# ethz-asl/object_keypoints

Measured on AMD Instinct MI355X. Metric: frames/sec keypoint inference (511x511 -> heatmaps+3D), higher is better.
Workload: dtype bf16; 1 GPU; BASELINE configs[2]: batch=64/GPU synthetic 511x511 frames, bf16 activations+weights, fp32 accumulate, CornerNet-Squeeze K=3 (valve) random-init procedural weights; fp32 NCHW frames -> stem -> hourglass+heads; peak-NMS -> depth lifting -> object grouping on injected bump scenes (SURVEY 8(d), 1-2 objects/frame); frames_per_gpu=64, global_batch=64, parallelism=frame-dp1, resident_frame_batches=4

## Files before the change

object_keypoints_amd/csrc/okp_igemm_patch.hip:

```cpp
#include <cstdio>
#include <cstdlib>
#include <cstring>
#include <type_traits>
#include <vector>

#include "okp_igemm_kernel.h"


namespace {

constexpr uint32_t kPatchKeys = 0x7ac788u;
template <int MT> __device__ __forceinline__ uint32_t patch_key(int col) {
  return MT == 16 ? (kPatchKeys >> (3 * (col >> 1))) & 7u : (uint32_t)(col >> 1) & 7u;
}

constexpr int kWStage = 256 * 128;
constexpr int kPitch = 18;
constexpr int kPatchBuf = 41 * 1024;
constexpr int kLdsPatch = 2 * kWStage;
constexpr int kLdsSteps = kLdsPatch + 2 * kPatchBuf;
constexpr int kLdsBias = kLdsSteps + 256 * (int)sizeof(OkpPatchStep);
#ifdef OKP_PATCH_STAMPS
constexpr int kStampBytes = 1024;
__device__ __forceinline__ uint64_t stamp() { uint64_t t; asm volatile("s_memtime %0" : "=s"(t)); return t; }
#else
constexpr int kStampBytes = 0;
#endif
constexpr int kGeoEntries = 328;
constexpr int kLdsGeo = kLdsBias + 1024;
constexpr int kLdsStamps = kLdsGeo + OKP_PATCH_MAX_GEOM * kGeoEntries * 4;
constexpr int kLdsTotal = kLdsStamps + kStampBytes;
static_assert(sizeof(OkpPatchStep) == 16, "step table entries are read as one 16-byte vector");
static_assert(256 * 512 <= kLdsSteps, "epilogue staging (256 px x 256 ch bf16) must not reach the step table");
static_assert(kLdsTotal <= 160 * 1024, "one workgroup's LDS is at most the CU's 160 KiB");

template <typename T, int MT = 16, bool RG = false>
__global__ __launch_bounds__(512) void okp_igemm_patch_kernel(const OkpPatchParams p) {
  static_assert(!RG || std::is_same<T, _Float16>::value, "the 16-bit storage guard is an fp16 instantiation");
  using x4_t = typename H16<T>::x4;
  using x8_t = typename H16<T>::x8;
  static_assert(MT == 16 || MT == 32, "MFMA tile");
  constexpr int TCO = 64 / MT, TPX = 128 / MT;
  constexpr int AREGS = MT * MT / 64;
  using acc_t = typename Mma<T, MT>::acc_t;
  __shared__ __attribute__((aligned(16))) char smem[kLdsTotal];
  char* const steps_lds = smem + kLdsSteps;
  char* const bias_lds = smem + kLdsBias;

  const int tid = threadIdx.x;
  const int lane = tid & 63;
  const int wave = __builtin_amdgcn_readfirstlane(tid >> 6);
  const int wco = wave >> 1, wpx = wave & 1;
  const int fr = lane & 15, fh = lane >> 4;

  const __amdgpu_buffer_rsrc_t rs_w = __builtin_amdgcn_make_buffer_rsrc(const_cast<void*>(p.weights), 0, (int)p.w_bytes, 0x00020000);
  const __amdgpu_buffer_rsrc_t rs_b = __builtin_amdgcn_make_buffer_rsrc(const_cast<float*>(p.bias), 0, p.n_co_tiles * 256 * 4, 0x00020000);
  const __amdgpu_buffer_rsrc_t rs_s0 = __builtin_amdgcn_make_buffer_rsrc(const_cast<void*>(p.src_data[0]), 0, (int)p.src_bytes[0], 0x00020000);
  const __amdgpu_buffer_rsrc_t rs_s1 = __builtin_amdgcn_make_buffer_rsrc(const_cast<void*>(p.src_data[1]), 0, (int)p.src_bytes[1], 0x00020000);

  if (tid < p.n_steps) reinterpret_cast<u32x4*>(steps_lds)[tid] = reinterpret_cast<const u32x4*>(p.steps)[tid];
  __syncthreads();

  const int r0 = tid >> 3;
  const int wc = (tid & 7) ^ ((r0 >> 1) & 7);

  for (int slot = blockIdx.x; slot < p.n_tiles; slot += gridDim.x) {
    const int xq = p.n_tiles >> 3, xr = p.n_tiles & 7, xcd = slot & 7;
    const int tile = (xcd < xr ? xcd * (xq + 1) : xr * (xq + 1) + (xcd - xr) * xq) + (slot >> 3);
    const int cls = p.n_classes == 4 ? (tile & 3) : 0;
    const int tile_c = p.n_classes == 4 ? (tile >> 2) : tile;
    const int t0 = cls * p.steps_per_class, t1 = t0 + p.steps_per_class;
    const int co_tile = tile_c % p.n_co_tiles;
    const int px_tile = tile_c / p.n_co_tiles;
    const int n = fastdiv(px_tile, p.div_tiles_frame);
    const int trem = px_tile - n * p.tiles_y * p.tiles_x;
    const int tyi = fastdiv(trem, p.div_tiles_x);
    const int y0 = tyi * 16, x0 = (trem - tyi * p.tiles_x) * 16;
    const int co0 = co_tile * 256;

    if (wave == 0)
      __builtin_amdgcn_raw_ptr_buffer_load_lds(rs_b, (lds_ptr_t)bias_lds, 16, (int)((uint32_t)(co0 + lane * 4) * 4u), 0, 0, 0);

    uint32_t wbase[4];
#pragma unroll
    for (int i = 0; i < 4; ++i) {
      const int co = co0 + r0 + i * 64;
      wbase[i] = (co < p.cout_pad) ? (uint32_t)co * 128u + (uint32_t)wc * 16u : kInvalidOff;
    }

    auto issue_w = [&](int t, int stage) {
      const uint32_t wslice = (uint32_t)t * (uint32_t)p.cout_pad * 128u;
      char* const wt = smem + stage * kWStage + wave * 1024;
#pragma unroll
      for (int i = 0; i < 4; ++i)
        __builtin_amdgcn_raw_ptr_buffer_load_lds(rs_w, (lds_ptr_t)(wt + i * 8192), 16, (int)(wbase[i] + wslice), 0, 0, 0);
    };
    auto patch_pixel = [&](const OkpPatchGeom& G, int idx) -> uint32_t {
      const int i = idx / kPitch, j = idx - i * kPitch;
      const int ys = G.conv_stride * y0 + G.oy + i * G.step, xs = G.conv_stride * x0 + G.ox + j * G.step;
      const bool ok = idx < G.npx && j < G.PW && ys >= 0 && ys < G.H && xs >= 0 && xs < G.W;
      return ok ? ((uint32_t)((n * G.H + ys) * G.W + xs) * (uint32_t)(G.pix_stride * 2)) | patch_key<MT>(j) : kInvalidOff;
    };
    auto issue_patch_tab = [&](int geom, uint32_t c0b, int k0, int k1, int buf) {
      const int npx = 18 * (int)((p.geom_ph >> (5 * geom)) & 31u);
      const __amdgpu_buffer_rsrc_t rs_x = ((p.geom_src >> geom) & 1) ? rs_s1 : rs_s0;
      const uint32_t* const tab = reinterpret_cast<const uint32_t*>(smem + kLdsGeo) + geom * kGeoEntries + (lane >> 3);
      for (int k = k0; k < k1; ++k) {
        const int blk = k * 8 + wave;
        if (blk * 8 >= npx) continue;
        const uint32_t e = tab[blk * 8];
        const uint32_t off = (e & kInvalidOff) ? kInvalidOff : (e & ~7u) + c0b + ((((uint32_t)lane & 7u) ^ (e & 7u)) << 4);
        __builtin_amdgcn_raw_ptr_buffer_load_lds(rs_x, (lds_ptr_t)(smem + kLdsPatch + buf * kPatchBuf + blk * 1024), 16, (int)off, 0, 0, 0);
      }
    };
    auto issue_patch = [&](int geom, uint32_t c0b, int k0, int k1, int buf) {
      const OkpPatchGeom& G = p.g[geom];
      const int PW = G.PW, npx = G.npx;
      const int H = G.H, W = G.W, ps2 = G.pix_stride * 2, step = G.step;
      const int yb = G.conv_stride * y0 + G.oy, xb = G.conv_stride * x0 + G.ox;
      const __amdgpu_buffer_rsrc_t rs_x = __builtin_amdgcn_make_buffer_rsrc(const_cast<void*>(G.data), 0, (int)G.bytes, 0x00020000);
      for (int k = k0; k < k1; ++k) {
        const int blk = k * 8 + wave;
        if (blk * 8 >= npx) continue;
        const int idx = blk * 8 + (lane >> 3);
        const int i = idx / kPitch, j = idx - i * kPitch;
        const int ch = (lane & 7) ^ (int)patch_key<MT>(j);
        const int ys = yb + i * step, xs = xb + j * step;
        const bool ok = idx < npx && j < PW && ys >= 0 && ys < H && xs >= 0 && xs < W;
        const uint32_t off = ok ? (uint32_t)((n * H + ys) * W + xs) * (uint32_t)ps2 + c0b + (uint32_t)ch * 16u : kInvalidOff;
        char* const dst = smem + kLdsPatch + buf * kPatchBuf + blk * 1024;
        __builtin_amdgcn_raw_ptr_buffer_load_lds(rs_x, (lds_ptr_t)dst, 16, (int)off, 0, 0, 0);
      }
    };

    acc_t acc[TCO][TPX];
#pragma unroll
    for (int i = 0; i < TCO; ++i)
#pragma unroll
      for (int j = 0; j < TPX; ++j)
#pragma unroll
        for (int e = 0; e < AREGS; ++e) acc[i][j][e] = 0.f;

    for (int g = 0; g < p.n_geom; ++g)
      if (tid < kGeoEntries) reinterpret_cast<uint32_t*>(smem + kLdsGeo)[g * kGeoEntries + tid] = patch_pixel(p.g[g], tid);
    {
      const u32x4 s0 = *reinterpret_cast<const u32x4*>(steps_lds + t0 * 16);
      const uint32_t w3 = (uint32_t)__builtin_amdgcn_readfirstlane((int)s0[3]);
      const int g0 = w3 & 0xff;
      issue_patch(g0, ((w3 >> 16) & 0xffu) * 128u, 0, (p.g[g0].npx + 63) >> 6, __builtin_amdgcn_readfirstlane((int)s0[2]) & 0xff);
    }
    issue_w(t0, t0 & 1);

    for (int t = t0; t < t1; ++t) {
      const u32x4 sv = *reinterpret_cast<const u32x4*>(steps_lds + t * 16);
      const uint32_t tap_bytes = (uint32_t)__builtin_amdgcn_readfirstlane((int)sv[0]);
      const uint32_t nx_c0b = (uint32_t)__builtin_amdgcn_readfirstlane((int)sv[1]);
      const uint32_t pk = (uint32_t)__builtin_amdgcn_readfirstlane((int)sv[2]);
      const int pbuf = pk & 0xff, nx_k0 = (pk >> 8) & 0xff, nx_k1 = (pk >> 16) & 0xff, nx_geom = pk >> 24;
      const uint32_t w3 = (uint32_t)__builtin_amdgcn_readfirstlane((int)sv[3]);
      const int dxo = (w3 >> 8) & 0xff;
      const bool more = t + 1 < t1;
#ifdef OKP_PATCH_ABL_NOPATCH
      const bool next_patch = false; (void)nx_k0; (void)nx_k1; (void)nx_geom; (void)nx_c0b;
#else
      const bool next_patch = nx_k1 > nx_k0 && (int)(w3 >> 24) + 1 < t1;
#endif

#ifdef OKP_PATCH_STAMPS
      uint64_t T0 = stamp();
      asm volatile("s_waitcnt vmcnt(0) lgkmcnt(0)" ::: "memory");
      uint64_t T1 = stamp();
      asm volatile("s_waitcnt lgkmcnt(0)" ::: "memory");
      __builtin_amdgcn_s_barrier();
      uint64_t T2 = stamp();
#else
      asm volatile("s_waitcnt vmcnt(0) lgkmcnt(0)" ::: "memory");
      __builtin_amdgcn_s_barrier();
#endif

      const char* const wt = smem + (t & 1) * kWStage;
      const char* const pbase = smem + kLdsPatch + pbuf * kPatchBuf;
      if constexpr (MT == 32) {
        const int r32 = lane & 31, h32 = lane >> 5;
        const char* const bb = pbase + tap_bytes + (uint32_t)(((wpx * 8 + (r32 >> 4)) * kPitch + (r32 & 15)) * 128);
        const uint32_t bsw = patch_key<32>((r32 & 15) + dxo);
        auto lda = [&](int sub, int i) { return *reinterpret_cast<const u32x4*>(wt + swz<128>((wco * TCO + i) * 32 + r32, 2 * sub + h32)); };
        auto ldb = [&](int sub, int j) { return *reinterpret_cast<const u32x4*>(bb + j * (2 * kPitch * 128) + ((((uint32_t)(2 * sub + h32)) ^ bsw) << 4)); };
        u32x4 fa[2][TCO], fb[2][TPX];
#pragma unroll
        for (int i = 0; i < TCO; ++i) fa[0][i] = lda(0, i);
#pragma unroll
        for (int j = 0; j < TPX; ++j) fb[0][j] = ldb(0, j);
        if (more) issue_w(t + 1, (t + 1) & 1);
#pragma unroll
        for (int sub = 0; sub < 4; ++sub) {
          __builtin_amdgcn_sched_barrier(0);
          if (sub + 1 < 4) {
#pragma unroll
            for (int i = 0; i < TCO; ++i) fa[(sub + 1) & 1][i] = lda(sub + 1, i);
#pragma unroll
            for (int j = 0; j < TPX; ++j) fb[(sub + 1) & 1][j] = ldb(sub + 1, j);
          }
          if (sub == 1 && next_patch) issue_patch_tab(nx_geom, nx_c0b, nx_k0, nx_k1, pbuf ^ 1);
          __builtin_amdgcn_sched_barrier(0);
#pragma unroll
          for (int i = 0; i < TCO; ++i)
#pragma unroll
            for (int j = 0; j < TPX; ++j) acc[i][j] = H16<T>::mfma32(fa[sub & 1][i], fb[sub & 1][j], acc[i][j]);
        }
      } else {
      const char* const bb = pbase + tap_bytes + (uint32_t)((wpx * TPX * kPitch + fr) * 128);
      const uint32_t bsw = patch_key<16>(fr + dxo);
      auto lda = [&](int kk, int i) {
        return *reinterpret_cast<const u32x4*>(wt + swz<128>((wco * TCO + i) * 16 + fr, 4 * kk + fh));
      };
      auto ldb = [&](int kk, int j) {
        return *reinterpret_cast<const u32x4*>(bb + j * (kPitch * 128) + ((((uint32_t)(4 * kk + fh)) ^ bsw) << 4));
      };
      auto mma8 = [&](const u32x4 (&a)[TCO], const u32x4 (&bq)[2], auto s) {
        constexpr int S = decltype(s)::value;
#pragma unroll
        for (int i = 0; i < TCO; ++i)
#pragma unroll
          for (int h = 0; h < 2; ++h)
            acc[i][2 * S + h] = H16<T>::mfma16(a[i], bq[h], acc[i][2 * S + h]);
      };
      using S0 = std::integral_constant<int, 0>; using S1 = std::integral_constant<int, 1>;
      using S2 = std::integral_constant<int, 2>; using S3 = std::integral_constant<int, 3>;
      u32x4 a0[TCO], a1[TCO], bq0[2], bq1[2];
#pragma unroll
      for (int i = 0; i < TCO; ++i) a0[i] = lda(0, i);
      bq0[0] = ldb(0, 0); bq0[1] = ldb(0, 1);
      bq1[0] = ldb(0, 2); bq1[1] = ldb(0, 3);
      if (more) issue_w(t + 1, (t + 1) & 1);
      __builtin_amdgcn_sched_barrier(0);
      mma8(a0, bq0, S0{});
      __builtin_amdgcn_sched_barrier(0);
#ifdef OKP_PATCH_STAMPS
      {
        uint64_t T3 = stamp();
        asm volatile("s_waitcnt lgkmcnt(0)" : "+s"(T0), "+s"(T1), "+s"(T2), "+s"(T3) :: "memory");
        if (slot == (int)blockIdx.x && lane == 0 && t - t0 < kStampBytes / 128)
          *reinterpret_cast<u32x4*>(smem + kLdsStamps + ((t - t0) * 8 + wave) * 16) = u32x4{(uint32_t)T0, (uint32_t)T1, (uint32_t)T2, (uint32_t)T3};
      }
      __builtin_amdgcn_sched_barrier(0);
#endif
      bq0[0] = ldb(0, 4); bq0[1] = ldb(0, 5); a1[0] = lda(1, 0); a1[1] = lda(1, 1);
      __builtin_amdgcn_sched_barrier(0);
      mma8(a0, bq1, S1{});
      __builtin_amdgcn_sched_barrier(0);
      bq1[0] = ldb(0, 6); bq1[1] = ldb(0, 7); a1[2] = lda(1, 2); a1[3] = lda(1, 3);
      __builtin_amdgcn_sched_barrier(0);
      mma8(a0, bq0, S2{});
      __builtin_amdgcn_sched_barrier(0);
      bq0[0] = ldb(1, 0); bq0[1] = ldb(1, 1);
      if (next_patch) issue_patch_tab(nx_geom, nx_c0b, nx_k0, nx_k1, pbuf ^ 1);
      __builtin_amdgcn_sched_barrier(0);
      mma8(a0, bq1, S3{});
      __builtin_amdgcn_sched_barrier(0);
      bq1[0] = ldb(1, 2); bq1[1] = ldb(1, 3);
      __builtin_amdgcn_sched_barrier(0);
      mma8(a1, bq0, S0{});
      __builtin_amdgcn_sched_barrier(0);
      bq0[0] = ldb(1, 4); bq0[1] = ldb(1, 5);
      __builtin_amdgcn_sched_barrier(0);
      mma8(a1, bq1, S1{});
      __builtin_amdgcn_sched_barrier(0);
      bq1[0] = ldb(1, 6); bq1[1] = ldb(1, 7);
      __builtin_amdgcn_sched_barrier(0);
      mma8(a1, bq0, S2{});
      mma8(a1, bq1, S3{});
          }
    }
#ifdef OKP_PATCH_STAMPS
    {
      uint64_t TE = stamp();
      asm volatile("s_waitcnt lgkmcnt(0)" : "+s"(TE) :: "memory");
      if (slot == (int)blockIdx.x && lane == 0 && t1 - t0 < kStampBytes / 128)
        *reinterpret_cast<u32x4*>(smem + kLdsStamps + ((t1 - t0) * 8 + wave) * 16) = u32x4{(uint32_t)TE, 0u, 0u, 0u};
    }
    __syncthreads();
    if (slot == (int)blockIdx.x && blockIdx.x < 16 && p.dbg)
      for (int i = tid; i < kStampBytes / 4; i += 512) p.dbg[blockIdx.x * (kStampBytes / 4) + i] = reinterpret_cast<const uint32_t*>(smem + kLdsStamps)[i];
#endif
    __syncthreads();

#pragma unroll
    for (int i = 0; i < TCO; ++i) {
#pragma unroll
      for (int g = 0; g < AREGS / 4; ++g) {
        const int co_l = (wco * TCO + i) * MT + (MT == 32 ? 8 * g + 4 * (lane >> 5) : 4 * fh);
        const f32x4 bv = *reinterpret_cast<const f32x4*>(bias_lds + co_l * 4);
#pragma unroll
        for (int j = 0; j < TPX; ++j) {
          const int prow = (wpx * TPX + j) * MT + (lane & (MT - 1));
          char* dst = smem + prow * 512 + ((((co_l * 2) >> 4) ^ (prow & 7)) << 4) + ((co_l * 2) & 15);
          x4_t o;
#pragma unroll
          for (int e = 0; e < 4; ++e) o[e] = (T)(acc[i][j][4 * g + e] + bv[e]);
          *reinterpret_cast<x4_t*>(dst) = o;
        }
      }
    }
    __syncthreads();
    constexpr int U = 256 * 32 / 512;
    constexpr int UH = 8;
    const bool relu = p.act == OKP_ACT_RELU;
    uint32_t range_h = 0u;
#pragma unroll 1
    for (int ub = 0; ub < U; ub += UH) {
      u32x4 rres[UH];
      uint32_t ooff[UH];
#pragma unroll
      for (int u = 0; u < UH; ++u) {
        const int it = tid + (ub + u) * 512;
        const int q = it & 31, prow = it >> 5;
        const int co = co0 + q * 8;
        const uint32_t opix = (uint32_t)((n * p.OH + (y0 + (prow >> 4)) * p.out_step + p.out_oy + (cls >> 1)) * p.OW + (x0 + (prow & 15)) * p.out_step + p.out_ox + (cls & 1));
        ooff[u] = co < p.cout ? opix : kInvalidOff;
      }
      if (p.res) {
#pragma unroll
        for (int u = 0; u < UH; ++u) {
          const int q = (tid + (ub + u) * 512) & 31;
          const int co = co0 + q * 8;
          const uint32_t opix = ooff[u] == kInvalidOff ? 0u : ooff[u];
          rres[u] = *reinterpret_cast<const u32x4*>(static_cast<const char*>(p.res) + ((size_t)opix * p.res_pix_stride + (co < p.cout ? co : 0)) * 2);
        }
      }
#pragma unroll
      for (int u = 0; u < UH; ++u) {
        const int it = tid + (ub + u) * 512;
        const int q = it & 31, prow = it >> 5;
        u32x4 w = *reinterpret_cast<const u32x4*>(smem + prow * 512 + ((q ^ (prow & 7)) << 4));
        if (ooff[u] == kInvalidOff) continue;
        char* op = static_cast<char*>(p.out) + ((size_t)ooff[u] * p.out_pix_stride + co0 + q * 8) * 2;
        if (!p.res) {
          if (relu) {
            typedef short s16x8 __attribute__((ext_vector_type(8)));
            const s16x8 z = {0, 0, 0, 0, 0, 0, 0, 0};
            w = __builtin_bit_cast(u32x4, __builtin_elementwise_max(__builtin_bit_cast(s16x8, w), z));
          }
          if constexpr (RG) range_h = okp_range_max_h8(range_h, w);
          *reinterpret_cast<u32x4*>(op) = w;
        } else {
          const x8_t s8 = __builtin_bit_cast(x8_t, w), r8 = __builtin_bit_cast(x8_t, rres[u]);
          x8_t o;
#pragma unroll
          for (int e = 0; e < 8; ++e) {
            float v = (float)s8[e] + (float)r8[e];
            if (relu) v = fmaxf(v, 0.f);
            o[e] = (T)v;
          }
          if constexpr (RG) range_h = okp_range_max_h8(range_h, __builtin_bit_cast(u32x4, o));
          *reinterpret_cast<x8_t*>(op) = o;
        }
      }
    }
    if constexpr (RG) okp_raise_range_flag(p.range_flag, okp_range_exceeded_h2(range_h));
    __syncthreads();
  }
}

}

bool okp_patch_supported(const okp_conv* plan, const OkpIgemmParams& p) {
  const bool x3 = plan->dtype == OKP_F32X3;
  if (!plan->patch_steps_dev || !(okp_is16(plan->dtype) || x3)) return false;
  if ((p.n_classes != 1 && p.n_classes != 4) || p.dw_w) return false;
  if (p.Ho % 16 || p.Wo % 16) return false;
  if (x3 && (p.out16 || p.res16 || p.out_sub2 || !p.out || plan->n_single_slices)) return false;
  for (int s = 0; s < plan->n_src; ++s) {
    if (p.src_pix_stride[s] < plan->cin[s]) return false;
    if ((p.src_pix_stride[s] * okp_esz(plan->dtype)) % 8) return false;
  }
  return true;
}

int okp_fill_patch_params(const okp_conv* plan, const OkpIgemmParams& q, OkpPatchParams& p) {
  std::memset(&p, 0, sizeof(p));
  for (int gi = 0; gi < plan->patch_n_geom; ++gi) {
    const int ss = plan->patch_src[gi];
    OkpPatchGeom& g = p.g[gi];
    g.data = q.src[ss]; g.bytes = q.src_bytes[ss]; g.H = q.srcH[ss]; g.W = q.srcW[ss]; g.pix_stride = q.src_pix_stride[ss];
    g.PW = plan->patch_PW[gi]; g.npx = 18 * plan->patch_PH[gi];
    g.oy = plan->patch_oy[gi]; g.ox = plan->patch_ox[gi]; g.step = plan->patch_step[gi]; g.conv_stride = plan->conv_stride[ss];
  }
  p.n_geom = plan->patch_n_geom;
  for (int gi = 0; gi < plan->patch_n_geom; ++gi) {
    const int ss = plan->patch_src[gi];
    const int64_t span = plan->dtype == OKP_F32X3 ? (int64_t)q.srcH[ss] * q.srcW[ss] * q.src_pix_stride[ss] * 4 : (q.src_bytes64[ss] ? q.src_bytes64[ss] : (int64_t)q.src_bytes[ss]);
    if (ss < 0 || ss > 1 || plan->patch_PH[gi] > 18 || span >= 0x7FFF0000ll) { okp_set_error("okp_conv_forward: patch geometry %d outside what the in-loop tables encode", gi); return OKP_EINVAL; }
    p.geom_ph |= (uint32_t)plan->patch_PH[gi] << (5 * gi);
    p.geom_src |= (uint32_t)ss << gi;
    p.src_data[ss] = q.src[ss]; p.src_bytes[ss] = q.src_bytes[ss];
    p.src_total_bytes[ss] = q.src_bytes64[ss] ? q.src_bytes64[ss] : (int64_t)q.src_bytes[ss];
    p.src_frame_bytes[ss] = (int64_t)q.srcH[ss] * q.srcW[ss] * q.src_pix_stride[ss] * okp_esz(plan->dtype);
  }
  if (!p.src_data[1]) { p.src_data[1] = p.src_data[0]; p.src_bytes[1] = p.src_bytes[0]; p.src_total_bytes[1] = p.src_total_bytes[0]; p.src_frame_bytes[1] = p.src_frame_bytes[0]; }
  p.weights = q.weights; p.w_bytes = q.w_bytes; p.cout_pad = q.cout_pad; p.cout = q.cout; p.bias = q.bias; p.oscale = q.oscale;
  p.steps = plan->patch_steps_dev; p.n_steps = plan->n_slices;
  p.n_classes = q.n_classes; p.steps_per_class = plan->n_slices / q.n_classes;
  p.OH = q.OH; p.OW = q.OW; p.out_step = q.out_step; p.out_oy = q.out_oy; p.out_ox = q.out_ox;
  p.N = q.N; p.H = q.Ho; p.W = q.Wo; p.tiles_y = q.Ho / 16; p.tiles_x = q.Wo / 16;
  p.div_tiles_frame = okp_fastdiv((uint32_t)(p.tiles_y * p.tiles_x)); p.div_tiles_x = okp_fastdiv((uint32_t)p.tiles_x);
  p.out = q.out; p.out_bytes = q.out_bytes; p.out_pix_stride = q.out_pix_stride;
  p.res = q.res; p.res_bytes = q.res_bytes; p.res_pix_stride = q.res_pix_stride; p.act = q.act;
  p.pairs = ((uint32_t)q.src_pairs & 3u) | (q.out_pairs ? 4u : 0u);
  p.range_flag = q.range_flag;
  p.n_co_tiles = q.cout_pad / 256;
  p.tiles_per_class = p.n_co_tiles * p.N * p.tiles_y * p.tiles_x;
  p.n_tiles = p.tiles_per_class * p.n_classes;
  return OKP_OK;
}

int okp_launch_igemm_patch(const okp_conv* plan, const OkpIgemmParams& q, hipStream_t stream) {
  if (!okp_patch_supported(plan, q)) { okp_set_error("okp_conv_forward: tile 13 (patch-resident kernel) does not apply to this plan / problem"); return OKP_EINVAL; }
  OkpPatchParams p;
  if (int e = okp_fill_patch_params(plan, q, p)) return e;
  if (plan->dtype == OKP_F32X3) return okp_launch_igemm_patch_x3(plan, p, stream);
#ifdef OKP_PATCH_STAMPS
  static uint32_t* dbg = nullptr;
  if (!dbg) (void)hipMalloc((void**)&dbg, 16 * kStampBytes);
  (void)hipMemsetAsync(dbg, 0, 16 * kStampBytes, stream);
  p.dbg = dbg;
#endif
  const dim3 grid((unsigned)(p.n_tiles < 256 ? p.n_tiles : 256)), block(512);
  if (q.mfma32) {
    if (plan->dtype == OKP_BF16) hipLaunchKernelGGL((okp_igemm_patch_kernel<__bf16, 32>), grid, block, 0, stream, p);
    else if (p.range_flag) hipLaunchKernelGGL((okp_igemm_patch_kernel<_Float16, 32, true>), grid, block, 0, stream, p);
    else hipLaunchKernelGGL((okp_igemm_patch_kernel<_Float16, 32>), grid, block, 0, stream, p);
  } else if (plan->dtype == OKP_BF16) hipLaunchKernelGGL((okp_igemm_patch_kernel<__bf16, 16>), grid, block, 0, stream, p);
  else if (p.range_flag) hipLaunchKernelGGL((okp_igemm_patch_kernel<_Float16, 16, true>), grid, block, 0, stream, p);
  else hipLaunchKernelGGL((okp_igemm_patch_kernel<_Float16, 16>), grid, block, 0, stream, p);
#ifdef OKP_PATCH_STAMPS
  if (getenv("OKP_PATCH_STAMPS_PRINT")) {
    (void)hipStreamSynchronize(stream);
    std::vector<uint32_t> h(16 * kStampBytes / 4);
    (void)hipMemcpy(h.data(), dbg, 16 * kStampBytes, hipMemcpyDeviceToHost);
    const int ns = std::min(p.steps_per_class, kStampBytes / 128 - 1);
    printf("patch stamps: %d K-steps per tile; clocks per step: wait for the LDS-DMA | barrier | until the first MFMA group was issued | rest of the body\n", p.steps_per_class);
    for (int wg = 0; wg < 16; wg += 5)
      for (int t = 0; t < ns; ++t) {
        printf("wg %2d step %2d:", wg, t);
        for (int w = 0; w < 8; w += 7) {
          const uint32_t* a = &h[(size_t)wg * (kStampBytes / 4) + (t * 8 + w) * 4];
          printf("   wave %d: %5u | %5u | %5u | %5u", w, a[1] - a[0], a[2] - a[1], a[3] - a[2], a[32] - a[3]);
        }
        printf("\n");
      }
    double sum[4] = {0, 0, 0, 0};
    int cnt = 0;
    for (int wg = 0; wg < 16; ++wg)
      for (int t = 1; t < ns; ++t)
        for (int w = 0; w < 8; ++w) {
          const uint32_t* a = &h[(size_t)wg * (kStampBytes / 4) + (t * 8 + w) * 4];
          sum[0] += a[1] - a[0]; sum[1] += a[2] - a[1]; sum[2] += a[3] - a[2]; sum[3] += a[32] - a[3]; ++cnt;
        }
    printf("mean over 16 workgroups, all waves, steps 1..: wait %.0f | barrier %.0f | first MFMAs %.0f | rest %.0f  = %.0f clocks per step\n",
           sum[0] / cnt, sum[1] / cnt, sum[2] / cnt, sum[3] / cnt, (sum[0] + sum[1] + sum[2] + sum[3]) / cnt);
  }
#endif
  return okp_check_hip(hipGetLastError(), "okp_igemm_patch launch");
}
```

object_keypoints_amd/csrc/okp_internal.h:

```cpp
#pragma once
#include <hip/hip_runtime.h>
#include <stdint.h>
#include "okp.h"

#define OKP_MAX_TAPS 32

typedef float f32x4 __attribute__((ext_vector_type(4)));
typedef float f32x16 __attribute__((ext_vector_type(16)));
typedef __bf16 bf16x8 __attribute__((ext_vector_type(8)));
typedef __bf16 bf16x4 __attribute__((ext_vector_type(4)));
typedef __bf16 bf16x2 __attribute__((ext_vector_type(2)));
typedef _Float16 f16x8 __attribute__((ext_vector_type(8)));
typedef _Float16 f16x4 __attribute__((ext_vector_type(4)));
typedef _Float16 f16x2 __attribute__((ext_vector_type(2)));
typedef unsigned int u32x4 __attribute__((ext_vector_type(4)));
typedef unsigned int u32x2 __attribute__((ext_vector_type(2)));

template <typename T> struct H16;
template <> struct H16<__bf16> {
  using x2 = bf16x2; using x4 = bf16x4; using x8 = bf16x8;
  static constexpr int kDtype = OKP_BF16;
  static __device__ __forceinline__ f32x4 mfma16(const u32x4& a, const u32x4& b, const f32x4& c) {
#if defined(__HIP_DEVICE_COMPILE__)
    return __builtin_amdgcn_mfma_f32_16x16x32_bf16(__builtin_bit_cast(bf16x8, a), __builtin_bit_cast(bf16x8, b), c, 0, 0, 0);
#else
    return c;
#endif
  }
  static __device__ __forceinline__ f32x16 mfma32(const u32x4& a, const u32x4& b, const f32x16& c) {
#if defined(__HIP_DEVICE_COMPILE__)
    return __builtin_amdgcn_mfma_f32_32x32x16_bf16(__builtin_bit_cast(bf16x8, a), __builtin_bit_cast(bf16x8, b), c, 0, 0, 0);
#else
    return c;
#endif
  }
  static __device__ __forceinline__ float lo(uint32_t w) { return __builtin_bit_cast(float, w << 16); }
  static __device__ __forceinline__ float hi(uint32_t w) { return __builtin_bit_cast(float, w & 0xffff0000u); }
};
template <> struct H16<_Float16> {
  using x2 = f16x2; using x4 = f16x4; using x8 = f16x8;
  static constexpr int kDtype = OKP_F16;
  static __device__ __forceinline__ f32x4 mfma16(const u32x4& a, const u32x4& b, const f32x4& c) {
#if defined(__HIP_DEVICE_COMPILE__)
    return __builtin_amdgcn_mfma_f32_16x16x32_f16(__builtin_bit_cast(f16x8, a), __builtin_bit_cast(f16x8, b), c, 0, 0, 0);
#else
    return c;
#endif
  }
  static __device__ __forceinline__ f32x16 mfma32(const u32x4& a, const u32x4& b, const f32x16& c) {
#if defined(__HIP_DEVICE_COMPILE__)
    return __builtin_amdgcn_mfma_f32_32x32x16_f16(__builtin_bit_cast(f16x8, a), __builtin_bit_cast(f16x8, b), c, 0, 0, 0);
#else
    return c;
#endif
  }
  static __device__ __forceinline__ float lo(uint32_t w) { return (float)__builtin_bit_cast(f16x2, w)[0]; }
  static __device__ __forceinline__ float hi(uint32_t w) { return (float)__builtin_bit_cast(f16x2, w)[1]; }
};

static __device__ __forceinline__ void okp_split4(const f32x4& x, u32x2& hi, u32x2& lo) {
#if defined(__HIP_DEVICE_COMPILE__)
#pragma unroll
  for (int q = 0; q < 2; ++q) {
    const float xa = x[2 * q], xb = x[2 * q + 1];
    f16x2 h2; h2[0] = (_Float16)xa; h2[1] = (_Float16)xb;
    const uint32_t hw = __builtin_bit_cast(uint32_t, h2);
    float da, db;
    asm("v_fma_mix_f32 %0, %1, -1.0, %2 op_sel:[0,0,0] op_sel_hi:[1,0,0]" : "=v"(da) : "v"(hw), "v"(xa));
    asm("v_fma_mix_f32 %0, %1, -1.0, %2 op_sel:[1,0,0] op_sel_hi:[1,0,0]" : "=v"(db) : "v"(hw), "v"(xb));
    f16x2 l2; l2[0] = (_Float16)da; l2[1] = (_Float16)db;
    hi[q] = hw; lo[q] = __builtin_bit_cast(uint32_t, l2);
  }
#else
  hi = u32x2{0u, 0u}; lo = u32x2{0u, 0u};
#endif
}

#ifdef OKP_NO_RANGE_GUARD
static __device__ __forceinline__ bool okp_unsplittable(float) { return false; }
static __device__ __forceinline__ float okp_range_max(float m, float) { return m; }
#else
static __device__ __forceinline__ bool okp_unsplittable(float v) { return !(__builtin_fabsf(v) <= 65504.f); }
static __device__ __forceinline__ float okp_range_max(float m, float v) { return __builtin_fmaxf(m, __builtin_fabsf(v)); }
#endif
static __device__ __forceinline__ bool okp_range_exceeded(float m) { return !(m <= 65504.f); }

typedef unsigned short okp_u16x2 __attribute__((ext_vector_type(2)));
#ifdef OKP_NO_RANGE_GUARD
static __device__ __forceinline__ uint32_t okp_range_max_h2(uint32_t m, uint32_t) { return m; }
#else
static __device__ __forceinline__ uint32_t okp_range_max_h2(uint32_t m, uint32_t w) {
  return __builtin_bit_cast(uint32_t, __builtin_elementwise_max(__builtin_bit_cast(okp_u16x2, m), __builtin_bit_cast(okp_u16x2, w & 0x7fff7fffu)));
}
#endif
static __device__ __forceinline__ uint32_t okp_range_max_h8(uint32_t m, const u32x4& w) {
#pragma unroll
  for (int i = 0; i < 4; ++i) m = okp_range_max_h2(m, w[i]);
  return m;
}
static __device__ __forceinline__ bool okp_range_exceeded_h2(uint32_t m) { return (m & 0xffffu) >= 0x7c00u || (m >> 16) >= 0x7c00u; }
static __device__ __forceinline__ void okp_raise_range_flag(int32_t* flag, bool bad) {
#if defined(__HIP_DEVICE_COMPILE__)
  if (flag != nullptr && bad) atomicOr(flag, 1);
#endif
}

template <typename T> __device__ __forceinline__ uint32_t okp_pack2(float a, float b) {
  typedef float f32x2_ __attribute__((ext_vector_type(2)));
  return __builtin_bit_cast(uint32_t, __builtin_convertvector((f32x2_){a, b}, typename H16<T>::x2));
}
inline int okp_esz(int dtype) { return (dtype == OKP_F32 || dtype == OKP_F32X3) ? 4 : 2; }
inline bool okp_is16(int dtype) { return dtype == OKP_BF16 || dtype == OKP_F16; }

struct OkpSlice {
  uint8_t tap_lo, tap_hi, src, nvalid;
  int32_t c0_lo, c0_hi;
  int32_t pad;
};

struct OkpTapDev {
  int32_t dy, dx, src, pad;
};

struct OkpFastDiv {
  uint32_t mul, shift;
};
inline OkpFastDiv okp_fastdiv(uint32_t d) {
  OkpFastDiv f{0u, 0u};
  if (d <= 1) return f;
  uint32_t s = 0;
  while ((1ull << s) < d) ++s;
  f.mul = (uint32_t)((1ull << (31 + s)) / d + 1);
  f.shift = s - 1;
  return f;
}

struct OkpIgemmParams {
  const void* src[2];
  uint32_t src_bytes[2];
  int32_t srcH[2], srcW[2], src_pix_stride[2], conv_stride[2];
  const void* weights;
  uint32_t w_bytes;
  int32_t cout_pad;
  const float* bias;
  const float* oscale;
  const OkpSlice* slices;
  int32_t n_slices;
  int32_t n_taps;
  int32_t N, Ho, Wo;
  OkpFastDiv div_howo, div_wo;
  void* out;
  uint32_t out_bytes, res_bytes;
  int32_t OH, OW, out_step, out_oy, out_ox, out_pix_stride;
  int32_t cout;
  const void* res;
  int32_t res_pix_stride;
  int32_t act;
  int32_t n_co_tiles;
  const float* dw_w;
  const float* dw_bias;
  void* dw_out;
  const void* dw_res;
  int32_t dw_out_pix_stride, dw_res_pix_stride;
  int32_t n_tiles;
  int32_t n_classes, tiles_per_class, slices_per_class;
  int32_t n_single_slices;
  void* out16;
  int32_t out16_pix_stride, res16;
  int32_t src_pairs, out_pairs;
  int32_t out_sub2, OH2, OW2;
  int32_t mfma32;
  int32_t* range_flag;
  int64_t src_bytes64[2];
  OkpTapDev taps[OKP_MAX_TAPS];
};

struct OkpPatchStep {
  uint32_t tap_bytes;
  uint32_t nx_c0b;
  uint8_t pbuf, nx_k0, nx_k1, nx_geom;
  uint8_t geom, tx, c0q, grp_last;
};
#define OKP_PSTEP_CVT_SELF 2u
#define OKP_PSTEP_CVT_NEXT 4u
#define OKP_PATCH_MAX_GEOM 6
static_assert(OKP_PATCH_MAX_GEOM * 5 <= 32, "OkpPatchParams.geom_ph packs 5 bits per geometry into one u32");
struct OkpPatchGeom {
  const void* data; uint32_t bytes;
  int32_t H, W, pix_stride;
  int32_t PW, npx;
  int32_t oy, ox;
  int32_t step, conv_stride;
};
struct OkpPatchParams {
  OkpPatchGeom g[OKP_PATCH_MAX_GEOM];
  int32_t n_geom;
  uint32_t geom_ph, geom_src;
  const void* src_data[2]; uint32_t src_bytes[2];
  const void* weights; uint32_t w_bytes; int32_t cout_pad, cout;
  const float* bias;
  const float* oscale;
  const OkpPatchStep* steps; int32_t n_steps;
  int32_t N, H, W, tiles_y, tiles_x;
  int32_t n_classes, steps_per_class, tiles_per_class;
  int32_t OH, OW, out_step, out_oy, out_ox;
  OkpFastDiv div_tiles_frame, div_tiles_x;
  void* out; uint32_t out_bytes; int32_t out_pix_stride;
  const void* res; uint32_t res_bytes; int32_t res_pix_stride;
  int32_t act, n_co_tiles, n_tiles;
  uint32_t pairs;
  int32_t* range_flag;
  int64_t src_total_bytes[2];
  int64_t src_frame_bytes[2];
#ifdef OKP_PATCH_STAMPS
  uint32_t* dbg;
#endif
};

struct OkpFire2Params {
  const void* x; uint32_t x_bytes; int32_t H, W, x_ps;
  void* out; uint32_t out_bytes; int32_t Ho, Wo, out_ps;
  int32_t N, skip;
  const void* w1; int32_t w1_cout_pad; const float* b1;
  const void* wa; int32_t wa_cout_pad; const float* ba;
  const float* wd; const float* bd;
  const float* s1; const float* sa;
  int32_t* range_flag;
  int32_t SH, SW, IH, IW, IP, RPR, tiles_y, tiles_x, n_tiles;
  OkpFastDiv div_tiles_frame, div_tiles_x, div_sw, div_iw, div_rpr;
#ifdef OKP_FIRE_STAMPS
  uint32_t* dbg;
#endif
};

struct OkpFireChainModule {
  const void* w1; int32_t w1_cout_pad; const float* b1;
  const void* wa; int32_t wa_cout_pad; const float* ba;
  const float* wd; const float* bd;
};
struct OkpFireChainParams {
  const void* x; void* out; int32_t x_ps, out_ps, H, W, n_modules;
  int32_t He, We;
  OkpFireChainModule mod[OKP_FIRE_CHAIN_MAX];
  int32_t* range_flag;
#ifdef OKP_FIRE_STAMPS
  uint32_t* dbg;
#endif
};

struct okp_conv {
  int dtype;
  int n_src;
  int32_t cin[2];
  int32_t conv_stride[2];
  int32_t cout, cout_pad;
  int32_t n_taps;
  OkpTapDev taps[OKP_MAX_TAPS];
  int32_t n_slices;
  int32_t n_single_slices;
  int act;
  void* weights_dev;
  uint32_t w_bytes;
  float* bias_dev;
  float* oscale_dev;
  OkpSlice* slices_dev;
  OkpPatchStep* patch_steps_dev;
  int32_t patch_n_geom;
  int32_t patch_src[OKP_PATCH_MAX_GEOM], patch_PW[OKP_PATCH_MAX_GEOM], patch_PH[OKP_PATCH_MAX_GEOM], patch_oy[OKP_PATCH_MAX_GEOM], patch_ox[OKP_PATCH_MAX_GEOM], patch_step[OKP_PATCH_MAX_GEOM];
  void* frag_dev;
  int32_t* range_flag;
  void* fragT_dev;
};

static __device__ __forceinline__ void okp_fisheye_undistort_point(const okp_camera& cam, double x, double y, double& xu, double& yu) {
  const double pwx = (x - cam.cx) / cam.fx, pwy = (y - cam.cy) / cam.fy;
  double theta_d = sqrt(pwx * pwx + pwy * pwy);
  const double half_pi = 1.5707963267948966;
  theta_d = fmin(fmax(-half_pi, theta_d), half_pi);
  double scale = 1.0;
  if (theta_d > 1e-8) {
    double theta = theta_d;
    for (int j = 0; j < 10; ++j) {
      const double t2 = theta * theta, t4 = t2 * t2, t6 = t4 * t2, t8 = t6 * t2;
      theta = theta_d / (1.0 + cam.d[0] * t2 + cam.d[1] * t4 + cam.d[2] * t6 + cam.d[3] * t8);
    }
    scale = tan(theta) / theta_d;
  }
  xu = cam.fx * (pwx * scale) + cam.cx;
  yu = cam.fy * (pwy * scale) + cam.cy;
}

static __device__ __forceinline__ void okp_radtan_undistort_point(const okp_camera& cam, double u, double v, double& xu, double& yu) {
  const double x0 = (u - cam.cx) / cam.fx, y0 = (v - cam.cy) / cam.fy;
  const double k1 = cam.d[0], k2 = cam.d[1], p1 = cam.d[2], p2 = cam.d[3];
  double x = x0, y = y0;
  for (int j = 0; j < 5; ++j) {
    const double r2 = x * x + y * y;
    const double icdist = 1.0 / (1.0 + (k2 * r2 + k1) * r2);
    const double dx = 2.0 * p1 * x * y + p2 * (r2 + 2.0 * x * x);
    const double dy = p1 * (r2 + 2.0 * y * y) + 2.0 * p2 * x * y;
    x = (x0 - dx) * icdist;
    y = (y0 - dy) * icdist;
  }
  xu = cam.fx * x + cam.cx;
  yu = cam.fy * y + cam.cy;
}

static __device__ __forceinline__ void okp_undistort_point(const okp_camera& cam, double x, double y, double& xu, double& yu) {
  if (cam.model == OKP_CAM_RADTAN) okp_radtan_undistort_point(cam, x, y, xu, yu);
  else okp_fisheye_undistort_point(cam, x, y, xu, yu);
}

static __device__ __forceinline__ void okp_lift_pixel(const okp_camera& cam, float x, float y, const float* __restrict__ depth, int W, int max_x, int max_y,
                                                      double& X, double& Y, double& Z) {
  double xu, yu;
  okp_undistort_point(cam, (double)x, (double)y, xu, yu);
  const float xf = (float)xu, yf = (float)yu;
  int xi = (int)rintf(xf), yi = (int)rintf(yf);
  xi = min(max(xi, 0), max_x);
  yi = min(max(yi, 0), max_y);
  const double z = (double)depth[(size_t)yi * W + xi];
  X = ((double)xf - cam.cx) / cam.fx * z;
  Y = ((double)yf - cam.cy) / cam.fy * z;
  Z = z;
}

void okp_set_error(const char* fmt, ...);
uint16_t okp_f32_to_16(int dtype, float f);
int okp_check_hip(hipError_t e, const char* what);

int okp_select_tile(int dtype, int cout_pad, long pixels);
int okp_launch_igemm(const okp_conv* plan, const OkpIgemmParams& p, int tile, hipStream_t stream);
int okp_ensure_frags(const okp_conv* plan, hipStream_t stream);
bool okp_fire2_supported(int cin, int mid, int half, int stride);
int okp_launch_fire2(int dtype, const OkpFire2Params& p, int cin, int mid, int stride, hipStream_t stream);
bool okp_fire_x3_supported(int cin, int mid, int half, int stride, int skip);
int okp_launch_fire_x3(OkpFire2Params p, int stride, hipStream_t stream);
bool okp_patch_supported(const okp_conv* plan, const OkpIgemmParams& p);
int okp_launch_igemm_patch(const okp_conv* plan, const OkpIgemmParams& p, hipStream_t stream);
int okp_fill_patch_params(const okp_conv* plan, const OkpIgemmParams& q, OkpPatchParams& p);
int okp_launch_igemm_patch_x3(const okp_conv* plan, const OkpPatchParams& p, hipStream_t stream);
```

Before: 12890 frames/s.

## Prefetch next tile's patch and bias during a split two-pass epilogue

The persistent implicit-GEMM patch kernel now splits the epilogue into two 128-pixel staging passes that live in the weight ring, which leaves the patch buffers free. While the output stores drain, it issues the next tile's geometry table, first patch DMA and bias load. On the first tile it also overlaps the step-table fill with the first loads instead of syncing up front. This hides per-tile prologue latency behind the epilogue, at the cost of more barriers, more complex control flow and an env toggle (OKP_PATCH_PREFETCH).

```diff
diff --git a/object_keypoints_amd/csrc/okp_igemm_patch.hip b/object_keypoints_amd/csrc/okp_igemm_patch.hip
--- a/object_keypoints_amd/csrc/okp_igemm_patch.hip
+++ b/object_keypoints_amd/csrc/okp_igemm_patch.hip
@@ -21,7 +21,11 @@
 constexpr int kLdsSteps = kLdsPatch + 2 * kPatchBuf;
 constexpr int kLdsBias = kLdsSteps + 256 * (int)sizeof(OkpPatchStep);
 #ifdef OKP_PATCH_STAMPS
-constexpr int kStampBytes = 1024;
+constexpr int kStepStampBytes = 1024;
+constexpr int kStampBytes = kStepStampBytes + 128;
+#ifndef OKP_PATCH_STAMPS_TILE
+#define OKP_PATCH_STAMPS_TILE 0
+#endif
 __device__ __forceinline__ uint64_t stamp() { uint64_t t; asm volatile("s_memtime %0" : "=s"(t)); return t; }
 #else
 constexpr int kStampBytes = 0;
@@ -31,7 +35,7 @@
 constexpr int kLdsStamps = kLdsGeo + OKP_PATCH_MAX_GEOM * kGeoEntries * 4;
 constexpr int kLdsTotal = kLdsStamps + kStampBytes;
 static_assert(sizeof(OkpPatchStep) == 16, "step table entries are read as one 16-byte vector");
-static_assert(256 * 512 <= kLdsSteps, "epilogue staging (256 px x 256 ch bf16) must not reach the step table");
+static_assert(128 * 512 <= kLdsPatch, "a staging pass (128 px x 256 ch, 16 bit) stays inside the weight ring: the patch buffers are live");
 static_assert(kLdsTotal <= 160 * 1024, "one workgroup's LDS is at most the CU's 160 KiB");
 
 template <typename T, int MT = 16, bool RG = false>
@@ -58,28 +62,77 @@
   const __amdgpu_buffer_rsrc_t rs_s0 = __builtin_amdgcn_make_buffer_rsrc(const_cast<void*>(p.src_data[0]), 0, (int)p.src_bytes[0], 0x00020000);
   const __amdgpu_buffer_rsrc_t rs_s1 = __builtin_amdgcn_make_buffer_rsrc(const_cast<void*>(p.src_data[1]), 0, (int)p.src_bytes[1], 0x00020000);
 
-  if (tid < p.n_steps) reinterpret_cast<u32x4*>(steps_lds)[tid] = reinterpret_cast<const u32x4*>(p.steps)[tid];
-  __syncthreads();
-
-  const int r0 = tid >> 3;
-  const int wc = (tid & 7) ^ ((r0 >> 1) & 7);
-
-  for (int slot = blockIdx.x; slot < p.n_tiles; slot += gridDim.x) {
+  struct Tile { int n, y0, x0, cls, t0, co0; };
+  auto tile_of = [&](int slot) -> Tile {
     const int xq = p.n_tiles >> 3, xr = p.n_tiles & 7, xcd = slot & 7;
     const int tile = (xcd < xr ? xcd * (xq + 1) : xr * (xq + 1) + (xcd - xr) * xq) + (slot >> 3);
     const int cls = p.n_classes == 4 ? (tile & 3) : 0;
     const int tile_c = p.n_classes == 4 ? (tile >> 2) : tile;
-    const int t0 = cls * p.steps_per_class, t1 = t0 + p.steps_per_class;
     const int co_tile = tile_c % p.n_co_tiles;
     const int px_tile = tile_c / p.n_co_tiles;
     const int n = fastdiv(px_tile, p.div_tiles_frame);
     const int trem = px_tile - n * p.tiles_y * p.tiles_x;
     const int tyi = fastdiv(trem, p.div_tiles_x);
-    const int y0 = tyi * 16, x0 = (trem - tyi * p.tiles_x) * 16;
-    const int co0 = co_tile * 256;
-
+    return Tile{n, tyi * 16, (trem - tyi * p.tiles_x) * 16, cls, cls * p.steps_per_class, co_tile * 256};
+  };
+
+  const u32x4 step0_g = *reinterpret_cast<const u32x4*>(p.steps + tile_of((int)blockIdx.x).t0);
+  u32x4 tabv = {0u, 0u, 0u, 0u};
+  if (tid < p.n_steps) tabv = reinterpret_cast<const u32x4*>(p.steps)[tid];
+  if (!p.prefetch) {
+    if (tid < p.n_steps) reinterpret_cast<u32x4*>(steps_lds)[tid] = tabv;
+    __syncthreads();
+  }
+
+  const int r0 = tid >> 3;
+  const int wc = (tid & 7) ^ ((r0 >> 1) & 7);
+
+  auto patch_pixel = [&](const OkpPatchGeom& G, const Tile& c, int idx) -> uint32_t {
+    const int i = idx / kPitch, j = idx - i * kPitch;
+    const int ys = G.conv_stride * c.y0 + G.oy + i * G.step, xs = G.conv_stride * c.x0 + G.ox + j * G.step;
+    const bool ok = idx < G.npx && j < G.PW && ys >= 0 && ys < G.H && xs >= 0 && xs < G.W;
+    return ok ? ((uint32_t)((c.n * G.H + ys) * G.W + xs) * (uint32_t)(G.pix_stride * 2)) | patch_key<MT>(j) : kInvalidOff;
+  };
+  auto issue_patch = [&](const Tile& c, int geom, uint32_t c0b, int k0, int k1, int buf) {
+    const OkpPatchGeom& G = p.g[geom];
+    const int PW = G.PW, npx = G.npx;
+    const int H = G.H, W = G.W, ps2 = G.pix_stride * 2, step = G.step;
+    const int yb = G.conv_stride * c.y0 + G.oy, xb = G.conv_stride * c.x0 + G.ox;
+    const __amdgpu_buffer_rsrc_t rs_x = __builtin_amdgcn_make_buffer_rsrc(const_cast<void*>(G.data), 0, (int)G.bytes, 0x00020000);
+    for (int k = k0; k < k1; ++k) {
+      const int blk = k * 8 + wave;
+      if (blk * 8 >= npx) continue;
+      const int idx = blk * 8 + (lane >> 3);
+      const int i = idx / kPitch, j = idx - i * kPitch;
+      const int ch = (lane & 7) ^ (int)patch_key<MT>(j);
+      const int ys = yb + i * step, xs = xb + j * step;
+      const bool ok = idx < npx && j < PW && ys >= 0 && ys < H && xs >= 0 && xs < W;
+      const uint32_t off = ok ? (uint32_t)((c.n * H + ys) * W + xs) * (uint32_t)ps2 + c0b + (uint32_t)ch * 16u : kInvalidOff;
+      char* const dst = smem + kLdsPatch + buf * kPatchBuf + blk * 1024;
+      __builtin_amdgcn_raw_ptr_buffer_load_lds(rs_x, (lds_ptr_t)dst, 16, (int)off, 0, 0, 0);
+    }
+  };
+  auto prepare = [&](const Tile& c, const u32x4& s0) {
+    for (int g = 0; g < p.n_geom; ++g)
+      if (tid < kGeoEntries) reinterpret_cast<uint32_t*>(smem + kLdsGeo)[g * kGeoEntries + tid] = patch_pixel(p.g[g], c, tid);
+    const uint32_t w3 = (uint32_t)__builtin_amdgcn_readfirstlane((int)s0[3]);
+    const int g0 = w3 & 0xff;
+    issue_patch(c, g0, ((w3 >> 16) & 0xffu) * 128u, 0, (p.g[g0].npx + 63) >> 6, __builtin_amdgcn_readfirstlane((int)s0[2]) & 0xff);
+  };
+  auto issue_bias = [&](const Tile& c) {
     if (wave == 0)
-      __builtin_amdgcn_raw_ptr_buffer_load_lds(rs_b, (lds_ptr_t)bias_lds, 16, (int)((uint32_t)(co0 + lane * 4) * 4u), 0, 0, 0);
+      __builtin_amdgcn_raw_ptr_buffer_load_lds(rs_b, (lds_ptr_t)bias_lds, 16, (int)((uint32_t)(c.co0 + lane * 4) * 4u), 0, 0, 0);
+  };
+
+  bool ready = false;
+  for (int slot = blockIdx.x; slot < p.n_tiles; slot += gridDim.x) {
+    const Tile cur = tile_of(slot);
+    const int n = cur.n, y0 = cur.y0, x0 = cur.x0, cls = cur.cls, co0 = cur.co0;
+    const int t0 = cur.t0, t1 = t0 + p.steps_per_class;
+    const bool first = slot == (int)blockIdx.x;
+#ifdef OKP_PATCH_STAMPS
+    const bool stamped = slot == (int)(blockIdx.x + OKP_PATCH_STAMPS_TILE * gridDim.x);
+#endif
 
     uint32_t wbase[4];
 #pragma unroll
@@ -94,12 +147,6 @@
 #pragma unroll
       for (int i = 0; i < 4; ++i)
         __builtin_amdgcn_raw_ptr_buffer_load_lds(rs_w, (lds_ptr_t)(wt + i * 8192), 16, (int)(wbase[i] + wslice), 0, 0, 0);
-    };
-    auto patch_pixel = [&](const OkpPatchGeom& G, int idx) -> uint32_t {
-      const int i = idx / kPitch, j = idx - i * kPitch;
-      const int ys = G.conv_stride * y0 + G.oy + i * G.step, xs = G.conv_stride * x0 + G.ox + j * G.step;
-      const bool ok = idx < G.npx && j < G.PW && ys >= 0 && ys < G.H && xs >= 0 && xs < G.W;
-      return ok ? ((uint32_t)((n * G.H + ys) * G.W + xs) * (uint32_t)(G.pix_stride * 2)) | patch_key<MT>(j) : kInvalidOff;
     };
     auto issue_patch_tab = [&](int geom, uint32_t c0b, int k0, int k1, int buf) {
       const int npx = 18 * (int)((p.geom_ph >> (5 * geom)) & 31u);
@@ -113,26 +160,6 @@
         __builtin_amdgcn_raw_ptr_buffer_load_lds(rs_x, (lds_ptr_t)(smem + kLdsPatch + buf * kPatchBuf + blk * 1024), 16, (int)off, 0, 0, 0);
       }
     };
-    auto issue_patch = [&](int geom, uint32_t c0b, int k0, int k1, int buf) {
-      const OkpPatchGeom& G = p.g[geom];
-      const int PW = G.PW, npx = G.npx;
-      const int H = G.H, W = G.W, ps2 = G.pix_stride * 2, step = G.step;
-      const int yb = G.conv_stride * y0 + G.oy, xb = G.conv_stride * x0 + G.ox;
-      const __amdgpu_buffer_rsrc_t rs_x = __builtin_amdgcn_make_buffer_rsrc(const_cast<void*>(G.data), 0, (int)G.bytes, 0x00020000);
-      for (int k = k0; k < k1; ++k) {
-        const int blk = k * 8 + wave;
-        if (blk * 8 >= npx) continue;
-        const int idx = blk * 8 + (lane >> 3);
-        const int i = idx / kPitch, j = idx - i * kPitch;
-        const int ch = (lane & 7) ^ (int)patch_key<MT>(j);
-        const int ys = yb + i * step, xs = xb + j * step;
-        const bool ok = idx < npx && j < PW && ys >= 0 && ys < H && xs >= 0 && xs < W;
-        const uint32_t off = ok ? (uint32_t)((n * H + ys) * W + xs) * (uint32_t)ps2 + c0b + (uint32_t)ch * 16u : kInvalidOff;
-        char* const dst = smem + kLdsPatch + buf * kPatchBuf + blk * 1024;
-        __builtin_amdgcn_raw_ptr_buffer_load_lds(rs_x, (lds_ptr_t)dst, 16, (int)off, 0, 0, 0);
-      }
-    };
-
     acc_t acc[TCO][TPX];
 #pragma unroll
     for (int i = 0; i < TCO; ++i)
@@ -141,15 +168,18 @@
 #pragma unroll
         for (int e = 0; e < AREGS; ++e) acc[i][j][e] = 0.f;
 
-    for (int g = 0; g < p.n_geom; ++g)
-      if (tid < kGeoEntries) reinterpret_cast<uint32_t*>(smem + kLdsGeo)[g * kGeoEntries + tid] = patch_pixel(p.g[g], tid);
-    {
-      const u32x4 s0 = *reinterpret_cast<const u32x4*>(steps_lds + t0 * 16);
-      const uint32_t w3 = (uint32_t)__builtin_amdgcn_readfirstlane((int)s0[3]);
-      const int g0 = w3 & 0xff;
-      issue_patch(g0, ((w3 >> 16) & 0xffu) * 128u, 0, (p.g[g0].npx + 63) >> 6, __builtin_amdgcn_readfirstlane((int)s0[2]) & 0xff);
+    if (!ready) {
+      issue_bias(cur);
+      u32x4 s0 = step0_g;
+      if (!(first && p.prefetch)) s0 = *reinterpret_cast<const u32x4*>(steps_lds + t0 * 16);
+      prepare(cur, s0);
     }
     issue_w(t0, t0 & 1);
+    if (first && p.prefetch) {
+      if (tid < p.n_steps) reinterpret_cast<u32x4*>(steps_lds)[tid] = tabv;
+      asm volatile("s_waitcnt lgkmcnt(0)" ::: "memory");
+      __builtin_amdgcn_s_barrier();
+    }
 
     for (int t = t0; t < t1; ++t) {
       const u32x4 sv = *reinterpret_cast<const u32x4*>(steps_lds + t * 16);
@@ -240,7 +270,7 @@
       {
         uint64_t T3 = stamp();
         asm volatile("s_waitcnt lgkmcnt(0)" : "+s"(T0), "+s"(T1), "+s"(T2), "+s"(T3) :: "memory");
-        if (slot == (int)blockIdx.x && lane == 0 && t - t0 < kStampBytes / 128)
+        if (stamped && lane == 0 && t - t0 < kStepStampBytes / 128)
           *reinterpret_cast<u32x4*>(smem + kLdsStamps + ((t - t0) * 8 + wave) * 16) = u32x4{(uint32_t)T0, (uint32_t)T1, (uint32_t)T2, (uint32_t)T3};
       }
       __builtin_amdgcn_sched_barrier(0);
@@ -273,69 +303,93 @@
           }
     }
 #ifdef OKP_PATCH_STAMPS
+    uint64_t E[5];
     {
       uint64_t TE = stamp();
       asm volatile("s_waitcnt lgkmcnt(0)" : "+s"(TE) :: "memory");
-      if (slot == (int)blockIdx.x && lane == 0 && t1 - t0 < kStampBytes / 128)
+      if (stamped && lane == 0 && t1 - t0 < kStepStampBytes / 128)
         *reinterpret_cast<u32x4*>(smem + kLdsStamps + ((t1 - t0) * 8 + wave) * 16) = u32x4{(uint32_t)TE, 0u, 0u, 0u};
     }
+#define OKP_EPI_STAMP(k) do { E[k] = stamp(); asm volatile("s_waitcnt lgkmcnt(0)" : "+s"(E[k]) :: "memory"); } while (0)
+#else
+#define OKP_EPI_STAMP(k) do { } while (0)
+#endif
     __syncthreads();
-    if (slot == (int)blockIdx.x && blockIdx.x < 16 && p.dbg)
-      for (int i = tid; i < kStampBytes / 4; i += 512) p.dbg[blockIdx.x * (kStampBytes / 4) + i] = reinterpret_cast<const uint32_t*>(smem + kLdsStamps)[i];
-#endif
-    __syncthreads();
-
-#pragma unroll
-    for (int i = 0; i < TCO; ++i) {
-#pragma unroll
-      for (int g = 0; g < AREGS / 4; ++g) {
-        const int co_l = (wco * TCO + i) * MT + (MT == 32 ? 8 * g + 4 * (lane >> 5) : 4 * fh);
-        const f32x4 bv = *reinterpret_cast<const f32x4*>(bias_lds + co_l * 4);
-#pragma unroll
-        for (int j = 0; j < TPX; ++j) {
-          const int prow = (wpx * TPX + j) * MT + (lane & (MT - 1));
-          char* dst = smem + prow * 512 + ((((co_l * 2) >> 4) ^ (prow & 7)) << 4) + ((co_l * 2) & 15);
-          x4_t o;
-#pragma unroll
-          for (int e = 0; e < 4; ++e) o[e] = (T)(acc[i][j][4 * g + e] + bv[e]);
-          *reinterpret_cast<x4_t*>(dst) = o;
-        }
-      }
-    }
-    __syncthreads();
-    constexpr int U = 256 * 32 / 512;
-    constexpr int UH = 8;
+    OKP_EPI_STAMP(0);
+
+    const int nslot = slot + (int)gridDim.x;
+    const bool pf = p.prefetch && nslot < p.n_tiles;
+    const Tile nx = tile_of(pf ? nslot : slot);
+    constexpr int UH = 128 * 32 / 512;
     const bool relu = p.act == OKP_ACT_RELU;
     uint32_t range_h = 0u;
-#pragma unroll 1
-    for (int ub = 0; ub < U; ub += UH) {
-      u32x4 rres[UH];
-      uint32_t ooff[UH];
+    u32x4 rres[UH];
+    uint32_t ooff[UH];
+    auto out_pixels = [&](int h, auto has_res) {
 #pragma unroll
       for (int u = 0; u < UH; ++u) {
-        const int it = tid + (ub + u) * 512;
-        const int q = it & 31, prow = it >> 5;
+        const int it = tid + u * 512;
+        const int q = it & 31, lr = it >> 5;
+        const int prow = (lr >> 6) * 128 + h * 64 + (lr & 63);
         const int co = co0 + q * 8;
         const uint32_t opix = (uint32_t)((n * p.OH + (y0 + (prow >> 4)) * p.out_step + p.out_oy + (cls >> 1)) * p.OW + (x0 + (prow & 15)) * p.out_step + p.out_ox + (cls & 1));
         ooff[u] = co < p.cout ? opix : kInvalidOff;
       }
-      if (p.res) {
+      if constexpr (decltype(has_res)::value) {
 #pragma unroll
         for (int u = 0; u < UH; ++u) {
-          const int q = (tid + (ub + u) * 512) & 31;
+          const int q = (tid + u * 512) & 31;
           const int co = co0 + q * 8;
           const uint32_t opix = ooff[u] == kInvalidOff ? 0u : ooff[u];
           rres[u] = *reinterpret_cast<const u32x4*>(static_cast<const char*>(p.res) + ((size_t)opix * p.res_pix_stride + (co < p.cout ? co : 0)) * 2);
         }
       }
+    };
+    auto passes = [&](auto has_res) {
+    constexpr bool RES = decltype(has_res)::value;
+#pragma unroll
+    for (int h = 0; h < 2; ++h) {
+      if (h == 1) out_pixels(1, has_res);
+#pragma unroll
+      for (int i = 0; i < TCO; ++i) {
+#pragma unroll
+        for (int g = 0; g < AREGS / 4; ++g) {
+          const int co_l = (wco * TCO + i) * MT + (MT == 32 ? 8 * g + 4 * (lane >> 5) : 4 * fh);
+          const f32x4 bv = *reinterpret_cast<const f32x4*>(bias_lds + co_l * 4);
+#pragma unroll
+          for (int jj = 0; jj < TPX / 2; ++jj) {
+            const int j = h * (TPX / 2) + jj;
+            const int lrow = (wpx * (TPX / 2) + jj) * MT + (lane & (MT - 1));
+            char* dst = smem + lrow * 512 + ((((co_l * 2) >> 4) ^ (lrow & 7)) << 4) + ((co_l * 2) & 15);
+            x4_t o;
+#pragma unroll
+            for (int e = 0; e < 4; ++e) o[e] = (T)(acc[i][j][4 * g + e] + bv[e]);
+            *reinterpret_cast<x4_t*>(dst) = o;
+          }
+        }
+      }
+      asm volatile("s_waitcnt lgkmcnt(0)" ::: "memory");
+      __builtin_amdgcn_s_barrier();
+      OKP_EPI_STAMP(1 + 2 * h);
+      if (h == 0) {
+        out_pixels(0, has_res);
+        if (!RES && pf) prepare(nx, *reinterpret_cast<const u32x4*>(steps_lds + nx.t0 * 16));
+      } else {
+        if constexpr (RES) __builtin_amdgcn_s_waitcnt(0x0F70);
+        if (pf) {
+          issue_bias(nx);
+          if (RES) prepare(nx, *reinterpret_cast<const u32x4*>(steps_lds + nx.t0 * 16));
+        }
+      }
 #pragma unroll
       for (int u = 0; u < UH; ++u) {
-        const int it = tid + (ub + u) * 512;
-        const int q = it & 31, prow = it >> 5;
-        u32x4 w = *reinterpret_cast<const u32x4*>(smem + prow * 512 + ((q ^ (prow & 7)) << 4));
-        if (ooff[u] == kInvalidOff) continue;
-        char* op = static_cast<char*>(p.out) + ((size_t)ooff[u] * p.out_pix_stride + co0 + q * 8) * 2;
-        if (!p.res) {
+        const int it = tid + u * 512;
+        const int q = it & 31, lr = it >> 5;
+        const uint32_t oo = ooff[u];
+        u32x4 w = *reinterpret_cast<const u32x4*>(smem + lr * 512 + ((q ^ (lr & 7)) << 4));
+        if (oo == kInvalidOff) continue;
+        char* op = static_cast<char*>(p.out) + ((size_t)oo * p.out_pix_stride + co0 + q * 8) * 2;
+        if constexpr (!RES) {
           if (relu) {
             typedef short s16x8 __attribute__((ext_vector_type(8)));
             const s16x8 z = {0, 0, 0, 0, 0, 0, 0, 0};
@@ -356,9 +410,23 @@
           *reinterpret_cast<x8_t*>(op) = o;
         }
       }
-    }
+      asm volatile("s_waitcnt lgkmcnt(0)" ::: "memory");
+      __builtin_amdgcn_s_barrier();
+      OKP_EPI_STAMP(2 + 2 * h);
+    }
+    };
+    if (p.res) passes(std::true_type{}); else passes(std::false_type{});
     if constexpr (RG) okp_raise_range_flag(p.range_flag, okp_range_exceeded_h2(range_h));
+    ready = pf;
+#ifdef OKP_PATCH_STAMPS
+    if (stamped && lane == 0)
+      *reinterpret_cast<u32x4*>(smem + kLdsStamps + kStepStampBytes + wave * 16) =
+          u32x4{(uint32_t)(E[1] - E[0]), (uint32_t)(E[2] - E[1]), (uint32_t)(E[3] - E[2]), (uint32_t)(E[4] - E[3])};
     __syncthreads();
+    if (stamped && blockIdx.x < 16 && p.dbg)
+      for (int i = tid; i < kStampBytes / 4; i += 512) p.dbg[blockIdx.x * (kStampBytes / 4) + i] = reinterpret_cast<const uint32_t*>(smem + kLdsStamps)[i];
+#endif
+#undef OKP_EPI_STAMP
   }
 }
 
@@ -419,6 +487,8 @@
   OkpPatchParams p;
   if (int e = okp_fill_patch_params(plan, q, p)) return e;
   if (plan->dtype == OKP_F32X3) return okp_launch_igemm_patch_x3(plan, p, stream);
+  static const bool prefetch_on = [] { const char* e = getenv("OKP_PATCH_PREFETCH"); return !(e && e[0] == '0'); }();
+  p.prefetch = prefetch_on ? 1 : 0;
 #ifdef OKP_PATCH_STAMPS
   static uint32_t* dbg = nullptr;
   if (!dbg) (void)hipMalloc((void**)&dbg, 16 * kStampBytes);
@@ -438,7 +508,7 @@
     (void)hipStreamSynchronize(stream);
     std::vector<uint32_t> h(16 * kStampBytes / 4);
     (void)hipMemcpy(h.data(), dbg, 16 * kStampBytes, hipMemcpyDeviceToHost);
-    const int ns = std::min(p.steps_per_class, kStampBytes / 128 - 1);
+    const int ns = std::min(p.steps_per_class, kStepStampBytes / 128 - 1);
     printf("patch stamps: %d K-steps per tile; clocks per step: wait for the LDS-DMA | barrier | until the first MFMA group was issued | rest of the body\n", p.steps_per_class);
     for (int wg = 0; wg < 16; wg += 5)
       for (int t = 0; t < ns; ++t) {
@@ -459,6 +529,16 @@
         }
     printf("mean over 16 workgroups, all waves, steps 1..: wait %.0f | barrier %.0f | first MFMAs %.0f | rest %.0f  = %.0f clocks per step\n",
            sum[0] / cnt, sum[1] / cnt, sum[2] / cnt, sum[3] / cnt, (sum[0] + sum[1] + sum[2] + sum[3]) / cnt);
+    double pro = 0, epi[4] = {0, 0, 0, 0};
+    for (int wg = 0; wg < 16; ++wg)
+      for (int w = 0; w < 8; ++w) {
+        const uint32_t* a = &h[(size_t)wg * (kStampBytes / 4) + w * 4];
+        const uint32_t* e = &h[(size_t)wg * (kStampBytes / 4) + kStepStampBytes / 4 + w * 4];
+        pro += a[1] - a[0];
+        for (int k = 0; k < 4; ++k) epi[k] += e[k];
+      }
+    printf("tile %d of each workgroup (prefetch %d), mean over 16 workgroups, all waves: prologue wait %.0f | staging 1 %.0f | stores 1 %.0f | staging 2 %.0f | stores 2 %.0f clocks\n",
+           OKP_PATCH_STAMPS_TILE, p.prefetch, pro / 128, epi[0] / 128, epi[1] / 128, epi[2] / 128, epi[3] / 128);
   }
 #endif
   return okp_check_hip(hipGetLastError(), "okp_igemm_patch launch");
diff --git a/object_keypoints_amd/csrc/okp_internal.h b/object_keypoints_amd/csrc/okp_internal.h
--- a/object_keypoints_amd/csrc/okp_internal.h
+++ b/object_keypoints_amd/csrc/okp_internal.h
@@ -210,6 +210,7 @@
   int32_t act, n_co_tiles, n_tiles;
   uint32_t pairs;
   int32_t* range_flag;
+  int32_t prefetch;
   int64_t src_total_bytes[2];
   int64_t src_frame_bytes[2];
 #ifdef OKP_PATCH_STAMPS
```

Result: no change. 13130 frames/s, median of 3 (+1.8%).
